# ubc-vision/joint-regressor-refinement

Measured on AMD Instinct MI355X. Metric: pose-refinement iters/sec, batch 4096, at 1/2/4/8 MI355X, higher is better.
Workload: dtype f32

## Files before the change

### joint-regressor-refinement_amd/build.py

```python
from __future__ import annotations

import argparse
import os
import subprocess
import sys
from concurrent.futures import ThreadPoolExecutor

HERE = os.path.dirname(os.path.abspath(__file__))
CSRC = os.path.join(HERE, 'csrc')
OBJ = os.path.join(HERE, 'build')
LIB = os.path.join(HERE, 'libjrr_hip.so')
SOURCES = ['api.hip', 'model.hip', 'refine.hip', 'prep.hip', 'lbs.hip', 'gemm.hip', 'disc.hip', 'eval.hip', 'fold.hip', 'sil.hip', 'sup.hip', 'image.hip', 'report.hip', 'shade.hip', 'export.hip', 'evalrep.hip', 'smooth.hip', 'regrep.hip', 'views.hip', 'accel.hip', 'jfit.hip', 'jmom.hip', 'jnorm.hip']
HEADERS = ['jrr_common.h', 'kernels.h', 'engine.h', 'dconv.h', 'supk.h', 'proj.h', 'rot6.h', 'quat.h', 'evalk.h', 'jfitk.h', os.path.join('..', '..', 'include', 'jrr.h')]
FLAGS = ['--offload-arch=gfx950', '-O3', '-fPIC', '-std=c++17', '-Wall', '-Wno-unused-function']


def _hipcc() -> str:
    for c in (os.environ.get('HIPCC'), '/opt/rocm/bin/hipcc', 'hipcc'):
        if c and (os.path.sep not in c or os.path.exists(c)):
            return c
    return 'hipcc'


def _stale(target: str, deps) -> bool:
# ... 78 lines not shown
                full = table[r['name']]
                depth, cut = 0, len(full)
                for i, ch in enumerate(full):
                    if ch == '<':
                        depth += 1
                    elif ch == '>':
                        depth -= 1
                    elif ch == '(' and depth == 0:
                        cut = i
                        break
                r['name'] = full[:cut].replace('void ', '', 1)
    return rows


def _waitcnt_parse(text: str):
    import re
    rows = []
    lines = text.splitlines()
    i = 0
    fn_re = re.compile(r'^(_Z\w+):')
    lab_re = re.compile(r'^(\.LBB\d+_\d+):(.*)$')
    while i < len(lines):
        m = fn_re.match(lines[i])
        if not m:
            i += 1
            continue
        name = m.group(1)
        i += 1
        blocks, cur = [], {'label': 'entry', 'loop': None, 'depth': 0, 'ins': []}
        last_label, sub, in_asm, hdr_depth = 'entry', 0, False, {}
        while i < len(lines) and not lines[i].startswith('.Lfunc_end'):
            ln = lines[i]
            i += 1
            lm = lab_re.match(ln)
            if lm:
                blocks.append(cur)
                label, note = lm.group(1), lm.group(2)
                loop, depth = None, 0
                h = re.search(r'Loop Header: Depth=(\d+)', note)
                if h:
                    loop, depth = label, int(h.group(1))
                    hdr_depth[label] = depth
                else:
                    h = re.search(r'in Loop: Header=(BB\d+_\d+) Depth=(\d+)', note)
                    if h:
                        loop, depth = '.L' + h.group(1), int(h.group(2))
                cur = {'label': label, 'loop': loop, 'depth': depth, 'ins': []}
                last_label, sub = label, 0
                continue
            s = ln.strip()
            if s.startswith(';;#ASMSTART'):
                in_asm = True
                continue
            if s.startswith(';;#ASMEND'):
                in_asm = False
                continue
            if not s or s.startswith(';') or s.startswith('.'):
                continue
            ins = s.split(';')[0].strip()
            if not ins:
                continue
            cur['ins'].append((ins, in_asm))
            b = re.match(r's_c?branch\w*\s+(\.LBB\d+_\d+)', ins)
            if b:
                blocks.append(cur)
                sub += 1
                loop, depth = cur['loop'], cur['depth']
                if loop is not None and b.group(1) == loop:
                    loop, depth = None, 0
                cur = {'label': f'{last_label}+{sub}', 'loop': loop, 'depth': depth, 'ins': []}
        blocks.append(cur)
        for blk in blocks:
            mfma = sum(1 for ins, _ in blk['ins'] if ins.startswith('v_mfma'))
            loads = sum(1 for ins, _ in blk['ins'] if re.match(r'(global|buffer|flat)_load', ins))
            for ins, ours in blk['ins']:
                if ours or not ins.startswith('s_waitcnt'):
                    continue
                v = re.search(r'vmcnt\((\d+)\)', ins)
                rows.append({'name': name, 'loop': blk['loop'], 'depth': blk['depth'], 'block': blk['label'], 'text': ins,
                             'vmcnt': int(v.group(1)) if v else None, 'mfma': mfma, 'loads': loads})
    return rows


def asm_load_hazards(asm: dict):
    import re
    out = []
    reg_re = re.compile(r'\bv\[(\d+):(\d+)\]|\bv(\d+)\b')

    def regs(operand_text):
        s = set()
        for m in reg_re.finditer(operand_text):
            if m.group(3) is not None:
                s.add(int(m.group(3)))
            else:
                s.update(range(int(m.group(1)), int(m.group(2)) + 1))
        return s

    for text in asm.values():
        lines = text.splitlines()
        starts = [i for i, ln in enumerate(lines) if re.match(r'^_Z\w+:', ln)]
        for fi, f0 in enumerate(starts):
            f1 = starts[fi + 1] if fi + 1 < len(starts) else len(lines)
            name = lines[f0].split(':')[0]
            body = lines[f0:f1]
            label_at = {m.group(1): k for k, ln in enumerate(body) for m in [re.match(r'^(\.LBB\d+_\d+):', ln)] if m}
            header_of = {}
            for k, ln in enumerate(body):
                m = re.match(r'^(\.LBB\d+_\d+):(.*)$', ln)
                if m:
                    h = re.search(r'in Loop: Header=(BB\d+_\d+)', m.group(2))
                    cur = '.L' + h.group(1) if h else (m.group(1) if 'Loop Header' in m.group(2) else None)
                header_of[k] = cur if m else header_of.get(k - 1)
            in_asm = False
            for k, ln in enumerate(body):
                s = ln.strip()
                if s.startswith(';;#ASMSTART'):
                    in_asm = True
                elif s.startswith(';;#ASMEND'):
                    in_asm = False
                m = re.match(r'global_load_dwordx4\s+v\[(\d+):(\d+)\]', s) if in_asm else None
                if not m:
                    continue
                tag = f'v[{m.group(1)}:{m.group(2)}]'
                dst = set(range(int(m.group(1)), int(m.group(2)) + 1))
                pos, wrapped, found, steps = k + 1, False, False, 0
                while pos < len(body) and steps < 20000:
                    steps += 1
                    t = body[pos].strip()
                    ins = t.split(';')[0].strip()
                    if t.startswith('s_waitcnt') and 'landed' in t and tag in t:
                        found = True
                        break
                    br = re.match(r's_c?branch\w*\s+(\.LBB\d+_\d+)', ins)
                    if br and ins.startswith('s_branch') and not wrapped and header_of.get(k) is not None:
                        tgt = label_at.get(br.group(1), len(body))
                        if tgt < pos and (br.group(1) == header_of[k] or header_of.get(tgt) == header_of[k]):
                            pos, wrapped = tgt, True
                            continue
                    if ins and not ins.startswith('.') and not re.match(r'^\.?\w+:', ins):
                        parts = ins.split(None, 1)
                        ops = parts[1] if len(parts) > 1 else ''
                        if regs(ops) & dst:
                            out.append(f'{name}: `{ins}` touches {tag} before its wait')
                    pos += 1
                if not found:
                    out.append(f'{name}: no `landed` wait for the load into {tag}')
    return out


def _summarise(out: str) -> str:
    import re
    rows, cur = [], None
    for line in out.splitlines():
        m = re.search(r'remark: Function Name: (\S+)', line)
        if m:
            name = m.group(1)
            try:
                name = subprocess.run(['c++filt', name], capture_output=True, text=True).stdout.strip() or name
            except OSError:
                pass
            cur = {'name': name.split('(')[0][:70]}
            rows.append(cur)
            continue
        for key, pat in (('vgpr', r'remark:\s+VGPRs: (\d+)'), ('agpr', r'AGPRs: (\d+)'), ('scratch', r'ScratchSize \[bytes/lane\]: (\d+)'),
                         ('occ', r'Occupancy \[waves/SIMD\]: (\d+)'), ('lds', r'LDS Size \[bytes/block\]: (\d+)'),
                         ('sgpr', r'remark:\s+SGPRs: (\d+)'), ('vspill', r'VGPRs Spill: (\d+)')):
# ... 79 lines not shown
```

### joint-regressor-refinement_amd/csrc/gemm.hip

```cpp
#include "jrr_common.h"
#include "kernels.h"

namespace jrr {


template <int WM, int WN, int WAVES_M, int WAVES_N, int GK, int EPI>
__global__ __launch_bounds__(64 * WAVES_M * WAVES_N) void k_gemm_tn(GemmArgs g) {
  constexpr int NW = WAVES_M * WAVES_N;
  constexpr int BM = 32 * WM * WAVES_M, BN = 32 * WN * WAVES_N;
  constexpr int A16 = GK * BM / 4, B16 = GK * BN / 4;
  constexpr int OPA = (A16 + 63) / 64, OPB = (B16 + 63) / 64;
  constexpr int PA = (OPA + NW - 1) / NW, PB = (OPB + NW - 1) / NW;
  constexpr int SLOT = GK * (BM + BN);
  __shared__ float lds[2 * SLOT];

  const int tid = threadIdx.x;
  const int wave = __builtin_amdgcn_readfirstlane(tid >> 6), lane = tid & 63, half = lane >> 5, l31 = lane & 31;
  const int wm = wave / WAVES_N, wn = wave % WAVES_N;
  const int n_mt = (g.M + BM - 1) / BM;
  const int L = xcd_remap(blockIdx.x, gridDim.x);
  const int mt = L % n_mt, nt = L / n_mt;
  const int m0 = mt * BM, n0 = nt * BN;
  const int nchunks = g.K / GK;
  const int split = blockIdx.z, nsplit = gridDim.z;
// ... 491 lines not shown
    for (int i = 0; i < 7; ++i) acc[i] = __builtin_amdgcn_mfma_f32_32x32x16_bf16(al[i], bh, acc[i], 0, 0, 0);
  }
  float* out = dFTp + (size_t)split * split_stride;
  const unsigned lane_off = (unsigned)(4 * half) * (unsigned)BP + (unsigned)(n0 + wave * 32 + l31);
#pragma unroll
  for (int i = 0; i < 7; ++i)
#pragma unroll
    for (int q = 0; q < 16; ++q) urow(out, (size_t)(32 * i + acc_row_u(q)), BP)[lane_off] = acc[i][q];
}
int launch_blend_adjoint_bf16x3(const void* Ds, const float* DVPq, float* dFTp, size_t split_stride, int BP, int nsplit, hipStream_t s) {
  hipLaunchKernelGGL(k_blend_adjoint_bf16x3, dim3(BP / 128, nsplit), dim3(256), 0, s, reinterpret_cast<const bf16x8*>(Ds), DVPq, dFTp, split_stride, BP);
  return 0;
}

template <int WM, int WAVES_M, int WAVES_N, int EPI, int BTR, int KS = 1>
__global__ __launch_bounds__(64 * WAVES_M * WAVES_N * KS) void k_disc_gemm(GemmArgs g) {
  constexpr int NW = WAVES_M * WAVES_N * KS, BM = 32 * WM * WAVES_M, BN = 32 * WAVES_N;
  constexpr int SA = 8 * BM * 4, SB = 8 * BN * 4, SLOT = SA + SB;
  constexpr int OPA = SA / 256, OPB = SB / 256, PA = OPA / NW, PB = OPB / NW;
  static_assert(OPA % NW == 0 && OPB % NW == 0, "exact tiling required");
  __shared__ __attribute__((aligned(16))) float lds[3 * SLOT];
  const int tid = threadIdx.x;
  const int wave = __builtin_amdgcn_readfirstlane(tid >> 6), lane = tid & 63, half = lane >> 5, l31 = lane & 31;
  const int ks = wave / (WAVES_M * WAVES_N), wpos = wave % (WAVES_M * WAVES_N);
  const int wm = wpos / WAVES_N, wn = wpos % WAVES_N;
  const int n_mt = g.M / BM;
  const int L = xcd_remap(blockIdx.x, gridDim.x);
  const int mt = L % n_mt, nt = L / n_mt;
  const int m0 = mt * BM, n0 = nt * BN;
  const int nch = g.K / 32;
  unsigned offA[PA], offB[PB];
#pragma unroll
  for (int i = 0; i < PA; ++i) {
    const int e = (wave + NW * i) * 64 + lane;
    offA[i] = ((unsigned)(e / BM) * (unsigned)g.M + (unsigned)(m0 + e % BM)) * 4u;
  }
#pragma unroll
  for (int i = 0; i < PB; ++i) {
    const int e = (wave + NW * i) * 64 + lane;
    offB[i] = ((unsigned)(e / BN) * (unsigned)g.ldb + (unsigned)(n0 + e % BN)) * 4u;
  }
  auto issue = [&](int ch, int slot) {
    const float* a = g.A + (size_t)ch * 8 * g.M * 4;
    const float* b = g.Bm + (size_t)ch * 8 * g.ldb * 4;
    asm volatile("" : "+s"(a));
    asm volatile("" : "+s"(b));
    float* dA = lds + slot * SLOT;
    float* dB = dA + SA;
#pragma unroll
    for (int i = 0; i < PA; ++i) __builtin_amdgcn_global_load_lds(JRR_GLB(a + offA[i]), JRR_LDS(dA + (wave + NW * i) * 256), 16, 0, 0);
#pragma unroll
    for (int i = 0; i < PB; ++i) __builtin_amdgcn_global_load_lds(JRR_GLB(b + offB[i]), JRR_LDS(dB + (wave + NW * i) * 256), 16, 0, 0);
  };
  issue(0, 0);
  if (nch > 1) issue(1, 1);
  float cscale = 0.f;
  if (BTR == 2) {
    const int n = n0 + wn * 32 + l31;
    constexpr int ZP = 16;
    float z = g.zbias[0];
    for (int t0 = 0; t0 < g.nzpart; t0 += ZP) {
      const int zlast = g.nzpart - 1 - t0;
      float zp[ZP];
#pragma unroll
      for (int t = 0; t < ZP; ++t) zp[t] = g.zpart[(size_t)(t0 + (t < zlast ? t : zlast)) * g.ldb + n];
#pragma unroll
      for (int t = 0; t < ZP; ++t) z = t <= zlast ? z + zp[t] : z;
    }
    const float sg = 1.f / (1.f + expf(-z));
    const bool ok = n < g.nvalid;
    const float up = g.gout ? (ok ? g.gout[(size_t)n * g.gout_ld] : 0.f) : g.scale * (sg - g.target);
    cscale = ok ? up * sg * (1.f - sg) : 0.f;
    if (mt == 0 && wm == 0 && half == 0 && ok) {
      if (g.sq0) g.sq0[n] = (sg - g.target) * (sg - g.target);
      if (g.out0) g.out0[(size_t)n * g.out0_ld] = sg;
    }
  }
  constexpr int NACC = (KS == 1) ? 2 : 1;
  f32x16 accs[NACC][WM];
#pragma unroll
  for (int a = 0; a < NACC; ++a)
#pragma unroll
    for (int i = 0; i < WM; ++i) accs[a][i] = zero16();
  int slot = 0;
  for (int ch = 0; ch < nch; ++ch) {
    if (ch + 1 < nch) asm volatile("s_waitcnt vmcnt(%0)" ::"n"(PA + PB) : "memory");
    else asm volatile("s_waitcnt vmcnt(0)" ::: "memory");
    __builtin_amdgcn_s_barrier();
    if (ch + 2 < nch) issue(ch + 2, slot >= 1 ? slot - 1 : 2);
    const f32x4* la = reinterpret_cast<const f32x4*>(lds + slot * SLOT) + wm * WM * 32 + l31;
    const f32x4* lb = reinterpret_cast<const f32x4*>(lds + slot * SLOT + SA) + wn * 32 + l31;
    slot = (slot == 2) ? 0 : slot + 1;
    constexpr int GQ = 4 / KS;
    const int gq0 = ks * GQ;
    f32x4 a4[WM], b4;
#pragma unroll
    for (int i = 0; i < WM; ++i) a4[i] = la[(2 * gq0 + half) * BM + 32 * i];
    b4 = lb[(2 * gq0 + half) * BN];
#pragma unroll
    for (int gq = 0; gq < GQ; ++gq) {
      f32x4 ca[WM], cb;
#pragma unroll
      for (int i = 0; i < WM; ++i) ca[i] = a4[i];
#pragma unroll
      for (int t = 0; t < 4; ++t) cb[t] = b4[t];
      f32x16 (&acc)[WM] = accs[(KS == 1) ? gq / 2 : 0];
      __builtin_amdgcn_sched_barrier(0);
      acc[0] = mfma(ca[0][0], cb[0], acc[0]);
      __builtin_amdgcn_sched_barrier(0);
      if (gq + 1 < GQ) {
#pragma unroll
        for (int i = 0; i < WM; ++i) a4[i] = la[(2 * (gq0 + gq) + 2 + half) * BM + 32 * i];
        b4 = lb[(2 * (gq0 + gq) + 2 + half) * BN];
      }
      __builtin_amdgcn_sched_barrier(0);
#pragma unroll
      for (int t = 0; t < 4; ++t)
#pragma unroll
        for (int i = 0; i < WM; ++i)
          if (t + i > 0) acc[i] = mfma(ca[i][t], cb[t], acc[i]);
    }
  }
  f32x16 (&acc)[WM] = accs[0];
  if (KS == 1) {
#pragma unroll
    for (int i = 0; i < WM; ++i) acc[i] += accs[NACC - 1][i];
  }
  if (KS == 2) {
    __syncthreads();
    float* red = lds + wpos * (WM * 16 * 64);
    if (ks == 1) {
#pragma unroll
      for (int i = 0; i < WM; ++i)
#pragma unroll
        for (int q = 0; q < 16; ++q) red[(i * 16 + q) * 64 + lane] = acc[i][q];
    }
    __syncthreads();
    if (ks == 1) return;
#pragma unroll
    for (int i = 0; i < WM; ++i)
#pragma unroll
      for (int q = 0; q < 16; ++q) acc[i][q] += red[(i * 16 + q) * 64 + lane];
  }
  const int n = n0 + wn * 32 + l31;
  float dot = 0.f;
  constexpr bool DOT_CHAIN = EPI == EPI_BIAS_RELU_DOT && WM == 1 && WAVES_M == 2 && WAVES_N == 1;
  float* const dotx = lds + 2 * (WM * 16 * 64) + 1024;
  if (DOT_CHAIN && wm == 1) { __syncthreads(); dot = dotx[lane]; }
#pragma unroll
  for (int i = 0; i < WM; ++i)
#pragma unroll
    for (int q4 = 0; q4 < 4; ++q4) {
      const int r0u = m0 + (wm * WM + i) * 32 + 8 * q4;
      const int r0 = r0u + 4 * half;
      f32x4 v = {acc[i][4 * q4], acc[i][4 * q4 + 1], acc[i][4 * q4 + 2], acc[i][4 * q4 + 3]};
      if (EPI == EPI_BIAS_RELU || EPI == EPI_BIAS_RELU_DOT) {
        const f32x4 bb = *reinterpret_cast<const f32x4*>(g.bias + r0);
#pragma unroll
        for (int u = 0; u < 4; ++u) v[u] = fmaxf(v[u] + bb[u], 0.f);
      }
      if (EPI == EPI_BIAS_RELU_DOT) {
        const f32x4 dw = *reinterpret_cast<const f32x4*>(g.dotw + r0);
#pragma unroll
        for (int u = 0; u < 4; ++u) dot = fmaf(dw[u], v[u], dot);
      }
      const size_t qi = ((size_t)(r0u / 4 + half) * g.ldo + n);
      if (EPI == EPI_MASK) {
        const f32x4 mk = reinterpret_cast<const f32x4*>(g.mask)[qi];
#pragma unroll
        for (int u = 0; u < 4; ++u) v[u] = (mk[u] > 0.f) ? (BTR == 2 ? v[u] * cscale : v[u]) : 0.f;
      }
      if (EPI == EPI_BIAS_RELU_DOT) {
#pragma unroll
        for (int u = 0; u < 4; ++u) v[u] = (v[u] > 0.f) ? 1.f : 0.f;
      }
      __builtin_nontemporal_store(v, &reinterpret_cast<f32x4*>(g.Out)[qi]);
    }
  if (DOT_CHAIN) {
    if (wm == 0) { dotx[lane] = dot; __syncthreads(); }
    else {
      const float t = dot + __shfl_xor(dot, 32);
      if (half == 0) g.dot_out[(size_t)mt * g.ldo + n] = t;
    }
  } else if (EPI == EPI_BIAS_RELU_DOT) {
    const float t = dot + __shfl_xor(dot, 32);
    if (half == 0) g.dot_out[(size_t)(mt * WAVES_M + wm) * g.ldo + n] = t;
  }
}

int launch_disc_gemm_q(const GemmArgs& g, int epi, int btr, hipStream_t s, int* ndot) {
  if (g.K % 32 != 0 || g.N % 64 != 0 || g.ldb % 4 != 0) { jrr_set_error("disc_gemm_q: unsupported shape M=%d N=%d K=%d", g.M, g.N, g.K); return JRR_ERR_ARG; }
  const bool t96 = g.M % 96 == 0 && (g.M % 128 != 0 || ((g.M / 128) * (g.N / 64) < 512 && (g.M / 96) * (g.N / 64) >= 512));
  if (!t96 && g.M % 128 != 0) { jrr_set_error("disc_gemm_q: M=%d is neither a multiple of 128 nor of 96", g.M); return JRR_ERR_ARG; }
  if (ndot) *ndot = t96 ? g.M / 96 : (g.M / 128) * 2;
  if (t96) {
    dim3 grid((g.M / 96) * (g.N / 64)), block(256);
    if (epi == EPI_STORE && !btr) hipLaunchKernelGGL((k_disc_gemm<3, 1, 2, EPI_STORE, 0, 2>), grid, block, 0, s, g);
    else { jrr_set_error("disc_gemm_q: 96-row tiles serve the plain store epilogue only"); return JRR_ERR_ARG; }
    return 0;
  }
  static const bool narrow_ok = [] { const char* e = getenv("JRR_DISC_NARROW"); return !(e && e[0] == '0'); }();
  if (narrow_ok && (g.M / 128) * (g.N / 64) < 512) {
    static const bool tiny_ok = [] { const char* e = getenv("JRR_DISC_NARROW"); return !(e && e[0] == '1'); }();
    if (tiny_ok && (g.M / 128) * (g.N / 32) < 512 && g.M % 64 == 0) {
      dim3 gridt((g.M / 64) * (g.N / 32)), blockt(256);
      if (epi == EPI_BIAS_RELU_DOT && !btr) hipLaunchKernelGGL((k_disc_gemm<1, 2, 1, EPI_BIAS_RELU_DOT, 0, 2>), gridt, blockt, 0, s, g);
      else if (epi == EPI_BIAS_RELU && !btr) hipLaunchKernelGGL((k_disc_gemm<1, 2, 1, EPI_BIAS_RELU, 0, 2>), gridt, blockt, 0, s, g);
      else if (epi == EPI_STORE && !btr) hipLaunchKernelGGL((k_disc_gemm<1, 2, 1, EPI_STORE, 0, 2>), gridt, blockt, 0, s, g);
      else if (epi == EPI_MASK && btr == 2) hipLaunchKernelGGL((k_disc_gemm<1, 2, 1, EPI_MASK, 2, 2>), gridt, blockt, 0, s, g);
      else { jrr_set_error("disc_gemm_q: unsupported epilogue %d / transform %d", epi, btr); return JRR_ERR_ARG; }
      return 0;
    }
    dim3 gridn((g.M / 128) * (g.N / 32)), blockn(256);
    if (epi == EPI_BIAS_RELU && !btr) hipLaunchKernelGGL((k_disc_gemm<2, 2, 1, EPI_BIAS_RELU, 0, 2>), gridn, blockn, 0, s, g);
    else if (epi == EPI_BIAS_RELU_DOT && !btr) hipLaunchKernelGGL((k_disc_gemm<2, 2, 1, EPI_BIAS_RELU_DOT, 0, 2>), gridn, blockn, 0, s, g);
    else if (epi == EPI_STORE && !btr) hipLaunchKernelGGL((k_disc_gemm<2, 2, 1, EPI_STORE, 0, 2>), gridn, blockn, 0, s, g);
    else if (epi == EPI_MASK && btr == 2) hipLaunchKernelGGL((k_disc_gemm<2, 2, 1, EPI_MASK, 2, 2>), gridn, blockn, 0, s, g);
    else { jrr_set_error("disc_gemm_q: unsupported epilogue %d / transform %d", epi, btr); return JRR_ERR_ARG; }
    return 0;
  }
  dim3 grid((g.M / 128) * (g.N / 64)), block(256);
  if (epi == EPI_BIAS_RELU && !btr) hipLaunchKernelGGL((k_disc_gemm<2, 2, 2, EPI_BIAS_RELU, 0>), grid, block, 0, s, g);
  else if (epi == EPI_BIAS_RELU_DOT && !btr) hipLaunchKernelGGL((k_disc_gemm<2, 2, 2, EPI_BIAS_RELU_DOT, 0>), grid, block, 0, s, g);
  else if (epi == EPI_STORE && !btr) hipLaunchKernelGGL((k_disc_gemm<2, 2, 2, EPI_STORE, 0>), grid, block, 0, s, g);
  else if (epi == EPI_MASK && btr == 2) hipLaunchKernelGGL((k_disc_gemm<2, 2, 2, EPI_MASK, 2>), grid, block, 0, s, g);
  else { jrr_set_error("disc_gemm_q: unsupported epilogue %d / transform %d", epi, btr); return JRR_ERR_ARG; }
  return 0;
}

__global__ void k_to_quads(const float* __restrict__ in, int ld, float* __restrict__ out, int K, int M) {
  const size_t i = (size_t)blockIdx.x * blockDim.x + threadIdx.x;
  if (i >= (size_t)K * M) return;
  const int k = (int)(i / M), m = (int)(i % M);
  out[((size_t)(k >> 2) * M + m) * 4 + (k & 3)] = in[(size_t)k * ld + m];
}
int launch_to_quads(const float* in, int ld, float* out, int K, int M, hipStream_t s) {
  hipLaunchKernelGGL(k_to_quads, dim3((unsigned)(((size_t)K * M + 255) / 256)), dim3(256), 0, s, in, ld, out, K, M);
  return 0;
}

}
```

### joint-regressor-refinement_amd/csrc/jrr_common.h

```cpp
#pragma once
#include <hip/hip_runtime.h>
#include <stdint.h>

#include <type_traits>
#include "../../include/jrr.h"

namespace jrr {

constexpr int V = 6890;
constexpr int VT = 216;
constexpr int VP = VT * 32;
constexpr int NJ = 24;
constexpr int NH = 17;
constexpr int NHP = 18;
constexpr int NB = 10;
constexpr int KF = 218;
constexpr int KFP = 224;
constexpr int KCH = 32;
constexpr int NKCH = KFP / KCH;
constexpr int BT = 32;
constexpr int BG = 128;
constexpr int FOLD_MJ = 512;
constexpr int FOLD_M = 1280;
constexpr int NPARAM = 154;
constexpr int KJS_MAX = 12;
constexpr int KJS_TILE_MAX = 16;

typedef float f32x16 __attribute__((ext_vector_type(16)));
typedef float f32x4 __attribute__((ext_vector_type(4)));

__device__ __forceinline__ f32x16 mfma(float a, float b, f32x16 c) {
  return __builtin_amdgcn_mfma_f32_32x32x2f32(a, b, c, 0, 0, 0);
}
__device__ __forceinline__ int acc_row(int reg, int half) { return (reg & 3) + 8 * (reg >> 2) + 4 * half; }

__device__ __forceinline__ f32x16 zero16() {
  f32x16 z;
#pragma unroll
  for (int i = 0; i < 16; ++i) z[i] = 0.f;
  return z;
}

__device__ __forceinline__ int xcd_remap(int id, int n) {
  int xcd = id & 7, q = n >> 3, r = n & 7;
  int base = (xcd < r) ? xcd * (q + 1) : r * (q + 1) + (xcd - r) * q;
  return base + (id >> 3);
}

#define JRR_LDS(p) ((__attribute__((address_space(3))) void*)(p))
#define JRR_GLB(p) ((const __attribute__((address_space(1))) void*)(p))

__device__ __forceinline__ float* urow(float* base, size_t row, int BP) {
  float* p = base + row * (size_t)BP;
  asm volatile("" : "+s"(p));
  return p;
}
__device__ __forceinline__ const float* urow(const float* base, size_t row, int BP) {
  const float* p = base + row * (size_t)BP;
  asm volatile("" : "+s"(p));
  return p;
}
__device__ __forceinline__ f32x4* quad_ptr(float* base, size_t plane_quad0, int g, int BP, unsigned lane_q) {
  float* p = base + ((plane_quad0 + 2 * g) * (size_t)BP) * 4;
  asm volatile("" : "+s"(p));
  return reinterpret_cast<f32x4*>(p) + lane_q;
}
__device__ __forceinline__ const f32x4* quad_ptr(const float* base, size_t plane_quad0, int g, int BP, unsigned lane_q) {
  const float* p = base + ((plane_quad0 + 2 * g) * (size_t)BP) * 4;
  asm volatile("" : "+s"(p));
  return reinterpret_cast<const f32x4*>(p) + lane_q;
}
__device__ __forceinline__ constexpr int acc_row_u(int q) { return (q & 3) + 8 * (q >> 2); }

template <int I, int N, class F>
__device__ __forceinline__ void static_for(F&& f) {
  if constexpr (I < N) {
    f(std::integral_constant<int, I>{});
    static_for<I + 1, N>(f);
  }
}

template <int N>
__device__ __forceinline__ void barrier_keep_vm() {
  static_assert(N >= 0 && N <= 63, "vmcnt is a 6-bit counter");
  asm volatile("s_waitcnt vmcnt(%0) lgkmcnt(0)\n\ts_barrier" ::"n"(N) : "memory");
}

template <bool NT>
__device__ __forceinline__ void quad_load(f32x4& dst, unsigned lane_off_bytes, const float* base_uniform) {
  if constexpr (NT) asm volatile("global_load_dwordx4 %0, %1, %2 nt" : "+v"(dst) : "v"(lane_off_bytes), "s"(base_uniform) : "memory");
  else asm volatile("global_load_dwordx4 %0, %1, %2" : "+v"(dst) : "v"(lane_off_bytes), "s"(base_uniform) : "memory");
}
template <int N>
__device__ __forceinline__ void quads_landed(f32x4 (&q)[3][2]) {
  static_assert(N >= 0 && N <= 63, "vmcnt is a 6-bit counter");
  asm volatile("s_waitcnt vmcnt(%6) ; landed %0 %1 %2 %3 %4 %5"
               : "+v"(q[0][0]), "+v"(q[0][1]), "+v"(q[1][0]), "+v"(q[1][1]), "+v"(q[2][0]), "+v"(q[2][1])
               : "n"(N));
}
template <int N>
__device__ __forceinline__ void quads_landed(f32x4 (&q)[3][2], f32x4 (&p)[3][2]) {
  static_assert(N >= 0 && N <= 63, "vmcnt is a 6-bit counter");
  asm volatile("s_waitcnt vmcnt(%12) ; landed %0 %1 %2 %3 %4 %5 %6 %7 %8 %9 %10 %11"
               : "+v"(q[0][0]), "+v"(q[0][1]), "+v"(q[1][0]), "+v"(q[1][1]), "+v"(q[2][0]), "+v"(q[2][1]),
                 "+v"(p[0][0]), "+v"(p[0][1]), "+v"(p[1][0]), "+v"(p[1][1]), "+v"(p[2][0]), "+v"(p[2][1])
               : "n"(N));
}

struct AdamScalars { float step_size, bc2_sqrt, beta1, beta2, eps; };
__device__ __forceinline__ AdamScalars adam_scalars(int step, float lr, float beta1, float beta2, float eps) {
  AdamScalars s;
  double bc1 = 1.0 - pow((double)beta1, (double)step);
  double bc2 = 1.0 - pow((double)beta2, (double)step);
  s.step_size = (float)((double)lr / bc1);
  s.bc2_sqrt = (float)sqrt(bc2);
  s.beta1 = beta1; s.beta2 = beta2; s.eps = eps;
  return s;
}
__device__ __forceinline__ float adam_update(float p, float g, float& m, float& v, const AdamScalars& s) {
  m = m * s.beta1 + (1.f - s.beta1) * g;
  v = v * s.beta2 + (1.f - s.beta2) * g * g;
  float denom = sqrtf(v) / s.bc2_sqrt + s.eps;
  return p - s.step_size * (m / denom);
}

struct Parents {
  int p[NJ];
  int depth[NJ];
  int maxd;
  unsigned char child_off[NJ + 1];
  unsigned char child[NJ];
};

struct Model {
  float* Dk;
  float* Dn;
  float* Dq;
  float* Wjv;
  float* Wvj;
  float* Wc;
  int* jl;
  int* tnj;
  int kjs;
  int wide_tiles, most_joints, permuted;
  int hint_applied;
  int tile_hist[NJ + 1];
  float* W16;
  int* segid;
  int* segj;
  int bwd16;
  int role_kjs;
  int* p2v;
  int* v2p;
// ... 40 lines not shown
```

### joint-regressor-refinement_amd/csrc/lbs.hip

```cpp
#include <cstdlib>

#include "jrr_common.h"
#include "kernels.h"

namespace jrr {

constexpr int W_FLOATS = NJ * 32;
constexpr int JN_FLOATS = 32 * 32;
constexpr int STG_FLOATS = KCH * 96 + KCH * BG;
constexpr int WJ_FLOATS = W_FLOATS + JN_FLOATS;
constexpr int NSTAGE = NKCH + 6;
constexpr int LBS_FWD_MFMA_PER_TILE = (KF / 2) * 3 + 6 * 24 + 3 * 16;
constexpr int TB_JN = 0, TB_WJV = NHP * 32, TB_WVJ = TB_WJV + W_FLOATS, TB_FLOATS = 2560;
constexpr int TB_W16_FLOATS = 16 * 36, TB_PIECES_SPARSE = 8;
constexpr int R16_JN = 0, R16_WT = 640, R16_WD = 1024, R16_JL = 1536, R16_WX = 1552, R16_FLOATS = 1792, R16_PIECES = 7;
__device__ __forceinline__ f32x16 mfma16(float a, float b, f32x16 c) { return __builtin_amdgcn_mfma_f32_16x16x1f32(a, b, c, 0, 0, 0); }

__device__ __forceinline__ void dma16(const float* gsrc_lane, float* lds_dst_wave) {
  __builtin_amdgcn_global_load_lds(JRR_GLB(gsrc_lane), JRR_LDS(lds_dst_wave), 16, 0, 0);
}
__device__ __forceinline__ void dma16u(const float* base_uniform, unsigned lane_off, float* lds_dst_wave) {
  asm volatile("" : "+s"(base_uniform));
  __builtin_amdgcn_global_load_lds(JRR_GLB(base_uniform + lane_off), JRR_LDS(lds_dst_wave), 16, 0, 0);
}
// ... 40 lines not shown
  const int wv = __builtin_amdgcn_readfirstlane(wave);
  const unsigned lane_rp = (unsigned)half * (unsigned)BP + (unsigned)l31 * 4u;
  const unsigned lane_ln = (unsigned)lane * 4u;
  const float* const Fbg = FT + (size_t)bg * BG * 4;
  const float* const Abg = AT + (size_t)bg * BG;
  unsigned lane_jl[2] = {0, 0};
  unsigned lane_jx[2] = {0, 0};
  int wide = 0, wide_next = 0;
  long long n_extra = 0;

  auto issue = [&](int vt, int s, int slot, int pass = 0, int wide_w = 0, int par = 0) {
    float* dst = ring + slot * STG_FLOATS;
    if (s < NKCH) {
      const float* dsrc = Dk + ((size_t)vt * KFP + s * KCH) * 96;
#pragma unroll
      for (int i = 0; i < 3; ++i) { const int o = wv + 4 * i; dma16u(dsrc + o * 256, lane_ln, dst + o * 256); }
      float* fdst = dst + KCH * 96;
#pragma unroll
      for (int i = 0; i < 4; ++i) {
        const int o = wv + 4 * i;
        dma16u(Fbg + ((size_t)(s * (KCH / 4) + (o >> 1)) * BP + (o & 1) * 64) * 4, lane_ln, fdst + o * 256);
      }
      if (s == 0) {
        float* wdst = wj + par * WJ_FLOATS;
        if (wv < ((SPARSE && wide_w) ? WT_COPIES_WIDE : WT_COPIES)) dma16u(Wjv + (size_t)vt * W_FLOATS + wv * 256, lane_ln, wdst + wv * 256);
        dma16u(Jn_vi + (size_t)vt * JN_FLOATS + wv * 256, lane_ln, wdst + W_FLOATS + wv * 256);
      }
    } else if (SPARSE) {
      const int r = s - NKCH;
      const unsigned o0 = pass ? lane_jx[0] : lane_jl[0], o1 = pass ? lane_jx[1] : lane_jl[1];
#pragma unroll
      for (int ci = 0; ci < 4; ++ci) {
        const int c = (ci == 0) ? 3 : ci - 1;
        dma16u(Abg + (size_t)((r * 4 + c) * NJ) * BP, o0, dst + ci * (KJS * BG) + wv * 256);
        if (KJS > 8 && wv < KJS / 2 - 4) dma16u(Abg + (size_t)((r * 4 + c) * NJ) * BP, o1, dst + ci * (KJS * BG) + (4 + wv) * 256);
      }
    } else {
      const int h = s - NKCH, r = h >> 1;
      const int c0 = (h & 1) ? 1 : 3, c1 = (h & 1) ? 2 : 0;
#pragma unroll
      for (int i = 0; i < 3; ++i) {
        const int o = wv + 4 * i;
        dma16u(Abg + (size_t)((r * 4 + c0) * NJ + 2 * o) * BP, lane_rp, dst + o * 256);
        dma16u(Abg + (size_t)((r * 4 + c1) * NJ + 2 * o) * BP, lane_rp, dst + NJ * BG + o * 256);
      }
    }
  };

  f32x16 jacc[3] = {zero16(), zero16(), zero16()};
  float j16[3] = {0.f, 0.f, 0.f};
  f32x16 vp[3];
  f32x16 vr;

  auto regress_operands = [&](const float* ldsJ, float (&ra)[4]) __attribute__((always_inline)) {
    const float* jp = ldsJ + half * 128 + (lane & 15);
#pragma unroll
    for (int q = 0; q < 4; ++q) ra[q] = jp[acc_row_u(q) * 32];
  };
  auto regress = [&](auto R_, const float* ldsJ, const float (&ra)[4]) __attribute__((always_inline)) {
    constexpr int r = decltype(R_)::value;
    const float* jp = ldsJ + half * 128 + (lane & 15);
    float a0 = ra[0], a1 = ra[1], a2 = ra[2], a3 = ra[3];
#pragma unroll
    for (int q = 0; q < 16; ++q) {
      const float ac = a0;
      a0 = a1; a1 = a2; a2 = a3;
      __builtin_amdgcn_sched_barrier(0);
      jacc[r] = mfma16(ac, vr[q], jacc[r]);
      __builtin_amdgcn_sched_barrier(0);
      if (q + 4 < 16) a3 = jp[acc_row_u(q + 4) * 32];
    }
    const float* sp = ldsJ + half * 128 + 16;
    float p16 = 0.f;
#pragma unroll
    for (int q = 0; q < 16; ++q) p16 = fmaf(sp[acc_row_u(q) * 32], vr[q], p16);
    j16[r] += p16;
  };

  auto pm_store = [&](int r, int vt, int g4, const f32x4& t) __attribute__((always_inline)) {
    const int ln = (int)__builtin_amdgcn_mbcnt_hi(~0u, __builtin_amdgcn_mbcnt_lo(~0u, 0u));
    const unsigned lo = ((unsigned)b0 + (unsigned)(ln & 31)) * (3u * VP) + 4u * (unsigned)(ln >> 5);
    float* base = VTb + ((size_t)r * VP + vt * 32 + 8 * g4);
    asm volatile("" : "+s"(base));
    *reinterpret_cast<f32x4*>(base + lo) = t;
  };
  const int t_first = (t_begin < t_end) ? (LIST ? tl[t_begin] : t_begin) : 0;
  if (SPARSE && WIDE && t_begin < t_end) wide_next = tnj[t_first] > KJS;
  if (t_begin < t_end) issue(t_first, 0, 0, 0, wide_next, t_begin & 1);
  int g = 0;
  for (int ix = t_begin; ix < t_end; ++ix) {
    const int vt = LIST ? tl[ix] : ix;
    const int vtn = LIST ? ((ix + 1 < t_end) ? tl[ix + 1] : 0) : ix + 1;
    const float* ldsW = wj + (ix & 1) * WJ_FLOATS;
    const float* ldsJ = ldsW + W_FLOATS;
    const bool stv = STORE_VERTS && (!vmask || vmask[vt] != 0);
    if (SPARSE) {
      if (WIDE) {
        wide = wide_next;
        wide_next = (ix + 1 < t_end) ? (tnj[vtn] > KJS) : 0;
      }
      const int j0 = jl[vt * NJ + 2 * wv], j1 = jl[vt * NJ + 2 * wv + 1];
      lane_jl[0] = (unsigned)(half ? j1 : j0) * (unsigned)BP + (unsigned)l31 * 4u;
      if (KJS > 8 && wv < KJS / 2 - 4) {
        const int j2 = jl[vt * NJ + 8 + 2 * wv], j3 = jl[vt * NJ + 8 + 2 * wv + 1];
        lane_jl[1] = (unsigned)(half ? j3 : j2) * (unsigned)BP + (unsigned)l31 * 4u;
      }
      if (WIDE && wide) {
        const int k0 = jl[vt * NJ + KJS + 2 * wv], k1 = jl[vt * NJ + KJS + 2 * wv + 1];
        lane_jx[0] = (unsigned)(half ? k1 : k0) * (unsigned)BP + (unsigned)l31 * 4u;
        if (KJS > 8 && wv < KJS / 2 - 4) {
          const int k2 = jl[vt * NJ + KJS + 8 + 2 * wv], k3 = jl[vt * NJ + KJS + 8 + 2 * wv + 1];
          lane_jx[1] = (unsigned)(half ? k3 : k2) * (unsigned)BP + (unsigned)l31 * 4u;
        }
        ++n_extra;
      }
    }
    static_for<0, NST>([&](auto S_) {
      constexpr int s = decltype(S_)::value;
      {
        constexpr int sp = (s == 0) ? NST - 1 : s - 1;
        constexpr int hp = sp - NKCH;
        constexpr int nst = (hp < 0) ? 0
                            : SPARSE ? (STORE_VP ? 4 : 0) + (STORE_VERTS ? 4 : 0)
                                     : (STORE_VP ? 2 : 0) + ((STORE_VERTS && (hp & 1)) ? 4 : 0);
        constexpr int nst_vp = (hp < 0) ? 0 : SPARSE ? (STORE_VP ? 4 : 0) : (STORE_VP ? 2 : 0);
        if (s == 0 && ix == t_begin) barrier_keep_vm<0>();
        else if (STORE_VERTS && nst != nst_vp && vmask) barrier_keep_vm<nst_vp>();
        else barrier_keep_vm<nst>();
      }
      if (SPARSE && WIDE && s >= NKCH && wide) issue(vt, s, (g + 1) & 1, 1);
      else if (s + 1 < NST) issue(vt, s + 1, (g + 1) & 1);
      else if (ix + 1 < t_end) issue(vtn, 0, (g + 1) & 1, 0, wide_next, (ix + 1) & 1);
      __builtin_amdgcn_sched_barrier(0);
      const float* buf = ring + (g & 1) * STG_FLOATS;
      if constexpr (s < NKCH) {
        if (s == 0) { vp[0] = zero16(); vp[1] = zero16(); vp[2] = zero16(); }
        constexpr int ngroups = 4;
        const f32x4* dq = reinterpret_cast<const f32x4*>(buf) + half * 96 + l31;
        const f32x4* fq = reinterpret_cast<const f32x4*>(buf + KCH * 96) + half * BG + wave * BT + l31;
        f32x4 a0 = dq[0], a1 = dq[32], a2 = dq[64], bq = fq[0];
        f32x4 n0 = a0, n1 = a1, n2 = a2, nb = bq;
#pragma unroll
        for (int gq = 0; gq < ngroups; ++gq) {
          constexpr int last_steps = KF - (NKCH - 1) * KCH - 24;
          const int nsteps = (s == NKCH - 1 && gq == ngroups - 1) ? last_steps : 4;
          const f32x4 c0 = a0, c1 = a1, c2 = a2, cb = bq;
          __builtin_amdgcn_sched_barrier(0);
          vp[0] = mfma(c0[0], cb[0], vp[0]);
          __builtin_amdgcn_sched_barrier(0);
          if (gq + 1 < ngroups) {
            n0 = dq[(2 * gq + 2) * 96]; n1 = dq[(2 * gq + 2) * 96 + 32]; n2 = dq[(2 * gq + 2) * 96 + 64];
            nb = fq[(2 * gq + 2) * BG];
          }
          __builtin_amdgcn_sched_barrier(0);
          vp[1] = mfma(c1[0], cb[0], vp[1]);
          vp[2] = mfma(c2[0], cb[0], vp[2]);
#pragma unroll
          for (int t = 1; t < 4; ++t) {
            if (t >= nsteps) break;
            vp[0] = mfma(c0[t], cb[t], vp[0]);
            vp[1] = mfma(c1[t], cb[t], vp[1]);
            vp[2] = mfma(c2[t], cb[t], vp[2]);
          }
          a0 = n0; a1 = n1; a2 = n2; bq = nb;
        }
      } else if constexpr (SPARSE) {
        constexpr int r = s - NKCH;
// ... 1228 lines not shown
```

Baseline: 893.4.

## Software-pipeline GEMM LDS reads across chunks, prefetch epilogue operands, use global address space

```diff
diff --git a/joint-regressor-refinement_amd/build.py b/joint-regressor-refinement_amd/build.py
--- a/joint-regressor-refinement_amd/build.py
+++ b/joint-regressor-refinement_amd/build.py
@@ -184,6 +184,203 @@
     return rows
 
 
+def _device_asm(sources=None):
+    import shutil
+    import tempfile
+    tmp = tempfile.mkdtemp(prefix='jrr_asm_')
+    names = list(sources or SOURCES)
+    jobs = [[_hipcc()] + FLAGS + ['--cuda-device-only', '-S', os.path.join(CSRC, src), '-o', os.path.join(tmp, src.replace('.hip', '.s'))]
+            for src in names]
+    try:
+        with ThreadPoolExecutor(max_workers=min(len(jobs), 8)) as ex:
+            outs = list(ex.map(lambda cmd: subprocess.run(cmd, capture_output=True, text=True), jobs))
+        asm = {}
+        for src, p in zip(names, outs):
+            if p.returncode != 0:
+                raise RuntimeError('hipcc failed:\n' + p.stderr[-2000:])
+            with open(os.path.join(tmp, src.replace('.hip', '.s'))) as f:
+                asm[src] = f.read()
+    finally:
+        shutil.rmtree(tmp, ignore_errors=True)
+    return asm
+
+
+def _demangled(mangled):
+    mangled = sorted(set(mangled))
+    try:
+        dem = subprocess.run(['c++filt'], input='\n'.join(mangled), capture_output=True, text=True).stdout.splitlines()
+    except OSError:
+        dem = []
+    if len(dem) != len(mangled):
+        return {m: m for m in mangled}
+    table = {}
+    for m, full in zip(mangled, dem):
+        depth, cut = 0, len(full)
+        for i, ch in enumerate(full):
+            if ch == '<':
+                depth += 1
+            elif ch == '>':
+                depth -= 1
+            elif ch == '(' and depth == 0:
+                cut = i
+                break
+        table[m] = full[:cut].replace('void ', '', 1)
+    return table
+
+
+def _functions(text: str):
+    import re
+    fn_re = re.compile(r'^(_Z\w+):')
+    lab_re = re.compile(r'^(\.LBB\d+_\d+):(.*)$')
+    lines = text.splitlines()
+    i = 0
+    while i < len(lines):
+        m = fn_re.match(lines[i])
+        i += 1
+        if not m:
+            continue
+        items, in_asm = [], False
+        while i < len(lines) and not lines[i].startswith('.Lfunc_end'):
+            ln = lines[i]
+            i += 1
+            lm = lab_re.match(ln)
+            if lm:
+                items.append(('label', (lm.group(1), lm.group(2))))
+                continue
+            s = ln.strip()
+            if s.startswith(';;#ASMSTART'):
+                in_asm = True
+            elif s.startswith(';;#ASMEND'):
+                in_asm = False
+            elif s and not s.startswith(';') and not s.startswith('.'):
+                ins = s.split(';')[0].strip()
+                if ins:
+                    items.append(('ins', (ins, in_asm)))
+        yield m.group(1), items
+
+
+def memory_rows(sources=None, asm=None):
+    import re
+    if asm is None:
+        asm = _device_asm(sources)
+    rows = []
+    for text in asm.values():
+        for name, items in _functions(text):
+            r = {'name': name, 'flat': 0, 'glob': 0, 'lds_dma': 0, 'lds': 0, 'flat_text': []}
+            for kind, (ins, _) in items:
+                if kind != 'ins':
+                    continue
+                op = ins.split()[0]
+                if op.startswith('flat_'):
+                    r['flat'] += 1
+                    r['flat_text'].append(ins)
+                elif op.startswith('global_load_lds') or (op.startswith('buffer_load') and re.search(r'\blds\b', ins)):
+                    r['lds_dma'] += 1
+                elif op.startswith('global_') or op.startswith('buffer_'):
+                    r['glob'] += 1
+                elif op.startswith('ds_'):
+                    r['lds'] += 1
+            rows.append(r)
+    table = _demangled(r['name'] for r in rows)
+    for r in rows:
+        r['name'] = table[r['name']]
+    return rows
+
+
+def lds_wait_rows(sources=None, asm=None):
+    import re
+    if asm is None:
+        asm = _device_asm(sources)
+    rows = []
+    for text in asm.values():
+        for name, items in _functions(text):
+            at_backedge, extents, label_at = {}, [], {}
+            announced = any(kind == 'label' and 'Loop Header' in payload[1] for kind, payload in items)
+            for emit in (False, True):
+                queue, nm, loop = [], 0, None
+                seen, fell = set(), True
+                for at, (kind, payload) in enumerate(items):
+                    if kind == 'label':
+                        label, note = payload
+                        seen.add(label)
+                        label_at[label] = at
+                        if 'Loop Header' in note:
+                            if not emit and fell and loop == label:
+                                at_backedge[label] = (list(queue), nm)
+                            loop = label
+                            if label in at_backedge:
+                                q, n0 = at_backedge[label]
+                                queue = [(d, c - n0 + nm) for d, c in q]
+                        else:
+                            h = re.search(r'in Loop: Header=(BB\d+_\d+)', note)
+                            loop = '.L' + h.group(1) if h else None
+                        continue
+                    ins, ours = payload
+                    op = ins.split()[0]
+                    fell = op != 's_branch'
+                    if op.startswith('v_mfma'):
+                        nm += 1
+                    elif op.startswith('ds_read'):
+                        queue.append((op, nm))
+                    elif op.startswith('ds_') or op.startswith('s_load') or op.startswith('s_buffer_load') or op.startswith('flat_'):
+                        queue.append((None, nm))
+                    elif op == 's_waitcnt':
+                        m = re.search(r'lgkmcnt\((\d+)\)', ins)
+                        if m:
+                            keep = int(m.group(1))
+                            waited = queue[:len(queue) - keep] if keep else queue
+                            reads = [c for d, c in waited if d]
+                            ops = [d for d, c in waited if d]
+                            inside = loop
+                            if inside is None and not announced:
+                                around = [e for e in extents if e[0] <= at <= e[1]]
+                                inside = min(around, key=lambda e: e[1] - e[0])[2] if around else None
+                            if emit and reads and not ours and inside is not None:
+                                rows.append({'name': name, 'loop': inside, 'text': ins, 'lgkmcnt': keep, 'reads': len(reads), 'ops': ops,
+                                             'mfma': nm - reads[0], 'mfma_youngest': nm - reads[-1]})
+                            queue = queue[len(queue) - keep:] if keep else []
+                    else:
+                        b = re.match(r's_c?branch\w*\s+(\.LBB\d+_\d+)', ins)
+                        if b and not emit and (b.group(1) in seen or b.group(1) == loop):
+                            at_backedge[b.group(1)] = (list(queue), nm)
+                            if b.group(1) in seen:
+                                extents.append((label_at[b.group(1)], at, b.group(1)))
+    table = _demangled(r['name'] for r in rows)
+    for r in rows:
+        r['name'] = table[r['name']]
+    return rows
+
+
+def overlapping_lds_reads(asm: dict):
+    import re
+    out = []
+    dst_re = re.compile(r'^ds_read\w*\s+v(?:\[(\d+):(\d+)\]|(\d+))')
+    reg_re = re.compile(r'\bv\[(\d+):(\d+)\]|\bv(\d+)\b')
+    for text in asm.values():
+        for name, items in _functions(text):
+            prev, waits, used = None, 0, False
+            for kind, payload in items:
+                if kind == 'label':
+                    prev = None
+                    continue
+                ins, ours = payload
+                m = dst_re.match(ins)
+                if m:
+                    lo, hi = (int(m.group(3)),) * 2 if m.group(3) is not None else (int(m.group(1)), int(m.group(2)))
+                    if prev and waits and not used and lo <= prev[2] and prev[1] <= hi:
+                        out.append(f'{name}: `{prev[0]}` and `{ins}` overlap, separated by a wait only')
+                    prev, waits, used = (ins, lo, hi), 0, False
+                elif prev:
+                    if ins.startswith('s_waitcnt'):
+                        waits += 0 if ours else 1
+                    else:
+                        for r in reg_re.finditer(ins.split(None, 1)[1] if ' ' in ins else ''):
+                            a, b = (int(r.group(3)),) * 2 if r.group(3) is not None else (int(r.group(1)), int(r.group(2)))
+                            if a <= prev[2] and prev[1] <= b:
+                                used = True
+    return out
+
+
 def asm_load_hazards(asm: dict):
     import re
     out = []
diff --git a/joint-regressor-refinement_amd/csrc/gemm.hip b/joint-regressor-refinement_amd/csrc/gemm.hip
--- a/joint-regressor-refinement_amd/csrc/gemm.hip
+++ b/joint-regressor-refinement_amd/csrc/gemm.hip
@@ -597,21 +597,26 @@
   for (int a = 0; a < NACC; ++a)
 #pragma unroll
     for (int i = 0; i < WM; ++i) accs[a][i] = zero16();
-  int slot = 0;
-  for (int ch = 0; ch < nch; ++ch) {
-    if (ch + 1 < nch) asm volatile("s_waitcnt vmcnt(%0)" ::"n"(PA + PB) : "memory");
-    else asm volatile("s_waitcnt vmcnt(0)" ::: "memory");
-    __builtin_amdgcn_s_barrier();
-    if (ch + 2 < nch) issue(ch + 2, slot >= 1 ? slot - 1 : 2);
-    const f32x4* la = reinterpret_cast<const f32x4*>(lds + slot * SLOT) + wm * WM * 32 + l31;
-    const f32x4* lb = reinterpret_cast<const f32x4*>(lds + slot * SLOT + SA) + wn * 32 + l31;
-    slot = (slot == 2) ? 0 : slot + 1;
-    constexpr int GQ = 4 / KS;
-    const int gq0 = ks * GQ;
-    f32x4 a4[WM], b4;
+  constexpr int GQ = 4 / KS;
+  const int gq0 = ks * GQ;
+  const int lao = wm * WM * 32 + l31, lbo = wn * 32 + l31;
+  f32x4 a4[WM], b4;
+  {
+    if (1 < nch) barrier_keep_vm<PA + PB>();
+    else barrier_keep_vm<0>();
+    if (2 < nch) issue(2, 2);
+    const f32x4* la = reinterpret_cast<const f32x4*>(lds) + lao;
+    const f32x4* lb = reinterpret_cast<const f32x4*>(lds + SA) + lbo;
 #pragma unroll
     for (int i = 0; i < WM; ++i) a4[i] = la[(2 * gq0 + half) * BM + 32 * i];
     b4 = lb[(2 * gq0 + half) * BN];
+  }
+  int slot = 0, ch = 0;
+  auto chunk = [&](auto LAST_) __attribute__((always_inline)) {
+    constexpr bool LAST = decltype(LAST_)::value;
+    const f32x4* la = reinterpret_cast<const f32x4*>(lds + slot * SLOT) + lao;
+    const f32x4* lb = reinterpret_cast<const f32x4*>(lds + slot * SLOT + SA) + lbo;
+    const int nslot = (slot == 2) ? 0 : slot + 1;
 #pragma unroll
     for (int gq = 0; gq < GQ; ++gq) {
       f32x4 ca[WM], cb;
@@ -627,6 +632,16 @@
 #pragma unroll
         for (int i = 0; i < WM; ++i) a4[i] = la[(2 * (gq0 + gq) + 2 + half) * BM + 32 * i];
         b4 = lb[(2 * (gq0 + gq) + 2 + half) * BN];
+      } else if (!LAST) {
+        if (ch + 2 < nch) barrier_keep_vm<PA + PB>();
+        else barrier_keep_vm<0>();
+        const f32x4* na = reinterpret_cast<const f32x4*>(lds + nslot * SLOT) + lao;
+        const f32x4* nb = reinterpret_cast<const f32x4*>(lds + nslot * SLOT + SA) + lbo;
+#pragma unroll
+        for (int i = 0; i < WM; ++i) a4[i] = na[(2 * gq0 + half) * BM + 32 * i];
+        b4 = nb[(2 * gq0 + half) * BN];
+        __builtin_amdgcn_sched_barrier(0);
+        if (ch + 3 < nch) issue(ch + 3, slot);
       }
       __builtin_amdgcn_sched_barrier(0);
 #pragma unroll
@@ -635,7 +650,10 @@
         for (int i = 0; i < WM; ++i)
           if (t + i > 0) acc[i] = mfma(ca[i][t], cb[t], acc[i]);
     }
-  }
+    slot = nslot;
+  };
+  for (; ch + 1 < nch; ++ch) chunk(std::false_type{});
+  if (ch < nch) chunk(std::true_type{});
   f32x16 (&acc)[WM] = accs[0];
   if (KS == 1) {
 #pragma unroll
@@ -661,27 +679,38 @@
   float dot = 0.f;
   constexpr bool DOT_CHAIN = EPI == EPI_BIAS_RELU_DOT && WM == 1 && WAVES_M == 2 && WAVES_N == 1;
   float* const dotx = lds + 2 * (WM * 16 * 64) + 1024;
+  f32x4 bbq[WM][4], dwq[WM][4], mkq[WM][4];
+  __builtin_amdgcn_sched_barrier(0);
+#pragma unroll
+  for (int i = 0; i < WM; ++i)
+#pragma unroll
+    for (int q4 = 0; q4 < 4; ++q4) {
+      const int r0u = m0 + (wm * WM + i) * 32 + 8 * q4, r0 = r0u + 4 * half;
+      if (EPI == EPI_BIAS_RELU || EPI == EPI_BIAS_RELU_DOT) bbq[i][q4] = *reinterpret_cast<const f32x4*>(g.bias + r0);
+      if (EPI == EPI_BIAS_RELU_DOT) dwq[i][q4] = *reinterpret_cast<const f32x4*>(g.dotw + r0);
+      if (EPI == EPI_MASK) mkq[i][q4] = reinterpret_cast<const f32x4*>(g.mask)[(size_t)(r0u / 4 + half) * g.ldo + n];
+    }
+  __builtin_amdgcn_sched_barrier(0);
   if (DOT_CHAIN && wm == 1) { __syncthreads(); dot = dotx[lane]; }
 #pragma unroll
   for (int i = 0; i < WM; ++i)
 #pragma unroll
     for (int q4 = 0; q4 < 4; ++q4) {
       const int r0u = m0 + (wm * WM + i) * 32 + 8 * q4;
-      const int r0 = r0u + 4 * half;
       f32x4 v = {acc[i][4 * q4], acc[i][4 * q4 + 1], acc[i][4 * q4 + 2], acc[i][4 * q4 + 3]};
       if (EPI == EPI_BIAS_RELU || EPI == EPI_BIAS_RELU_DOT) {
-        const f32x4 bb = *reinterpret_cast<const f32x4*>(g.bias + r0);
+        const f32x4 bb = bbq[i][q4];
 #pragma unroll
         for (int u = 0; u < 4; ++u) v[u] = fmaxf(v[u] + bb[u], 0.f);
       }
       if (EPI == EPI_BIAS_RELU_DOT) {
-        const f32x4 dw = *reinterpret_cast<const f32x4*>(g.dotw + r0);
+        const f32x4 dw = dwq[i][q4];
 #pragma unroll
         for (int u = 0; u < 4; ++u) dot = fmaf(dw[u], v[u], dot);
       }
       const size_t qi = ((size_t)(r0u / 4 + half) * g.ldo + n);
       if (EPI == EPI_MASK) {
-        const f32x4 mk = reinterpret_cast<const f32x4*>(g.mask)[qi];
+        const f32x4 mk = mkq[i][q4];
 #pragma unroll
         for (int u = 0; u < 4; ++u) v[u] = (mk[u] > 0.f) ? (BTR == 2 ? v[u] * cscale : v[u]) : 0.f;
       }
diff --git a/joint-regressor-refinement_amd/csrc/jrr_common.h b/joint-regressor-refinement_amd/csrc/jrr_common.h
--- a/joint-regressor-refinement_amd/csrc/jrr_common.h
+++ b/joint-regressor-refinement_amd/csrc/jrr_common.h
@@ -49,26 +49,27 @@
 
 #define JRR_LDS(p) ((__attribute__((address_space(3))) void*)(p))
 #define JRR_GLB(p) ((const __attribute__((address_space(1))) void*)(p))
+#define JRR_GPTR(T) __attribute__((address_space(1))) T*
 
-__device__ __forceinline__ float* urow(float* base, size_t row, int BP) {
+__device__ __forceinline__ JRR_GPTR(float) urow(float* base, size_t row, int BP) {
   float* p = base + row * (size_t)BP;
   asm volatile("" : "+s"(p));
-  return p;
+  return (JRR_GPTR(float))p;
 }
-__device__ __forceinline__ const float* urow(const float* base, size_t row, int BP) {
+__device__ __forceinline__ JRR_GPTR(const float) urow(const float* base, size_t row, int BP) {
   const float* p = base + row * (size_t)BP;
   asm volatile("" : "+s"(p));
-  return p;
+  return (JRR_GPTR(const float))p;
 }
-__device__ __forceinline__ f32x4* quad_ptr(float* base, size_t plane_quad0, int g, int BP, unsigned lane_q) {
+__device__ __forceinline__ JRR_GPTR(f32x4) quad_ptr(float* base, size_t plane_quad0, int g, int BP, unsigned lane_q) {
   float* p = base + ((plane_quad0 + 2 * g) * (size_t)BP) * 4;
   asm volatile("" : "+s"(p));
-  return reinterpret_cast<f32x4*>(p) + lane_q;
+  return (JRR_GPTR(f32x4))p + lane_q;
 }
-__device__ __forceinline__ const f32x4* quad_ptr(const float* base, size_t plane_quad0, int g, int BP, unsigned lane_q) {
+__device__ __forceinline__ JRR_GPTR(const f32x4) quad_ptr(const float* base, size_t plane_quad0, int g, int BP, unsigned lane_q) {
   const float* p = base + ((plane_quad0 + 2 * g) * (size_t)BP) * 4;
   asm volatile("" : "+s"(p));
-  return reinterpret_cast<const f32x4*>(p) + lane_q;
+  return (JRR_GPTR(const f32x4))p + lane_q;
 }
 __device__ __forceinline__ constexpr int acc_row_u(int q) { return (q & 3) + 8 * (q >> 2); }
 
diff --git a/joint-regressor-refinement_amd/csrc/lbs.hip b/joint-regressor-refinement_amd/csrc/lbs.hip
--- a/joint-regressor-refinement_amd/csrc/lbs.hip
+++ b/joint-regressor-refinement_amd/csrc/lbs.hip
@@ -146,7 +146,7 @@
     const unsigned lo = ((unsigned)b0 + (unsigned)(ln & 31)) * (3u * VP) + 4u * (unsigned)(ln >> 5);
     float* base = VTb + ((size_t)r * VP + vt * 32 + 8 * g4);
     asm volatile("" : "+s"(base));
-    *reinterpret_cast<f32x4*>(base + lo) = t;
+    *(JRR_GPTR(f32x4))(base + lo) = t;
   };
   const int t_first = (t_begin < t_end) ? (LIST ? tl[t_begin] : t_begin) : 0;
   if (SPARSE && WIDE && t_begin < t_end) wide_next = tnj[t_first] > KJS;
```

Result: faster. 904.2, median of 6 (+1.2%).
